# ketanfatania/QMRI-PnP-Recon-POC

Hardware: AMD Instinct MI355X
Metric: ADMM iters/sec (224x224x10 TSMI, spiral mask) (higher is better)
Workload: dtype f32; 1 GPU; cut3 224x224x10 single slice per GPU, spiral mask S=771 T=200, PnP-ADMM + 10-channel UNetRes (DRUNet) denoiser; solver=lsqr, admm_iters=20, dc_dtype=f64, parallelism=slice-parallel x1 (no collective)

## Files before the change

### qmri_pnp_recon_poc_amd/csrc/api_core.cpp

```cpp
#include "qmri_internal.h"
#include "fft_codelets.h"

#include <algorithm>
#include <atomic>
#include <cmath>
#include <cstdarg>
#include <cstdlib>
#include <cstring>
#include <mutex>

static thread_local std::string g_create_err;

namespace {
struct KnobDef { const char* name; int dflt; };
const KnobDef g_knob_defs[K_COUNT] = {
    {"conv_scheme", 2}, {"conv_f32", 0}, {"conv_wt", 1}, {"conv_xcd", 1}, {"conv_persist", 1}, {"conv_splitk", 1},
    {"conv_midcfg", 3}, {"conv_deepcfg", 3}, {"conv_deepks", 4},
    {"conv_resident", 1}, {"res_head", 1}, {"res_tail", 1}, {"res_down", 1}, {"res_delay", 24}, {"res_rearm", 64},
    {"res_stamps", 0}, {"conv_stamps", 0}, {"conv_stamp_launch", -1}, {"lsqr_stamps", 0},
    {"conv_mt2", 1024}, {"conv_occ", 2},
    {"fuse_ew", 1}, {"lsqr_persist", 1}, {"lsqr_fold", 1}, {"dictw_lsp", 2}, {"verbose", 0},
    {"pack_gpu", 1}, {"nufft_seg", NU_SEG},
};
std::atomic<int> g_knob_val[K_COUNT];
std::once_flag g_knob_once;

int knob_index(const char* name, size_t len) {
    for (int k = 0; k < K_COUNT; ++k)
        if (strlen(g_knob_defs[k].name) == len && strncmp(g_knob_defs[k].name, name, len) == 0) return k;
    return -1;
}
void knob_init() {
    for (int k = 0; k < K_COUNT; ++k) g_knob_val[k].store(g_knob_defs[k].dflt, std::memory_order_relaxed);
    const char* e = getenv("QMRI_DEBUG");
    while (e && *e) {
        const char* end = strchr(e, ',');
        const size_t len = end ? (size_t)(end - e) : strlen(e);
        const char* eq = (const char*)memchr(e, '=', len);
        const int k = eq ? knob_index(e, (size_t)(eq - e)) : -1;
        if (k >= 0) g_knob_val[k].store(atoi(eq + 1), std::memory_order_relaxed);
        else if (len) fprintf(stderr, "libqmri: QMRI_DEBUG: unknown or malformed entry '%.*s' ignored\n", (int)len, e);
// ... 829 lines not shown
```

### qmri_pnp_recon_poc_amd/csrc/api_net.cpp

```cpp
#include "qmri_internal.h"

#include <algorithm>
#include <cmath>
#include <cstdio>
#include <cstring>
#include <thread>
#include <chrono>
#include <cstdlib>

void qmri_free_operator(qmri_ctx* ctx);
int qmri_prepare_direct(qmri_ctx* ctx, double r);
int qmri_lsqr_run(qmri_ctx* ctx, int B, const double2* d_z, double r, double tol, int maxit, double2* d_x,
                  int32_t* iters_out, int32_t* flag_out, double* pdiag, LsqrState* hslot, bool* deferred, const LsqrFuse* fuse);

extern "C" size_t qmri_net_nparams(const qmri_net_desc* d) {
    if (!d) return 0;
    size_t n = 0;
    if (d->arch == QMRI_ARCH_UNETRES) {
        const int32_t* nc = d->nc;
        n += (size_t)nc[0] * d->in_nc * 9;
        for (int l = 0; l < 3; ++l) n += (size_t)2 * d->nb * nc[l] * nc[l] * 9 + (size_t)nc[l + 1] * nc[l] * 4;
        n += (size_t)2 * d->nb * nc[3] * nc[3] * 9;
        for (int l = 3; l > 0; --l) n += (size_t)nc[l] * nc[l - 1] * 4 + (size_t)2 * d->nb * nc[l - 1] * nc[l - 1] * 9;
        n += (size_t)d->out_nc * nc[0] * 9;
// ... 382 lines not shown
        for (int l = 0; l < 4; ++l) { p.x[l].blk = blk; p.a[l].blk = blk; p.t[l].blk = blk; }
    }
    const bool report = !ctx->net.force_f32;
    const bool timed = ctx->prof_level >= 2;
    if (timed) QMRI_HIP(ctx, hipEventRecord(ctx->ev[2], ctx->stream));
    if (report) QMRI_TRY(conv6_act_begin(ctx, (int)ctx->net.layers.size()));
    QMRI_TRY(net_forward_layers(ctx, B));
    if (report) QMRI_TRY(conv6_act_end(ctx));
    if (timed) QMRI_HIP(ctx, hipEventRecord(ctx->ev[3], ctx->stream));
    QMRI_TRY(qmri_prof_chain_finish(ctx));
    if (timed) {
        float ms = 0.f;
        QMRI_HIP(ctx, hipEventSynchronize(ctx->ev[3]));
        QMRI_HIP(ctx, hipEventElapsedTime(&ms, ctx->ev[2], ctx->ev[3]));
        ctx->prof.ms_net_forward += ms; ctx->prof.n_net_forward += 1;
    }
    return QMRI_OK;
}

static int net_forward_layers(qmri_ctx* ctx, int B) {
    NetPlan& p = ctx->net;
    const int nb = p.desc.nb;
    size_t li = 0;
    if (p.desc.arch == QMRI_ARCH_SEQ_CONV) {
        const size_t nl = p.layers.size();
        const PTensor* in = &p.in32;
        const PTensor* bufs[2] = { &p.a[0], &p.t[0] };
        for (size_t l = 0; l < nl; ++l) {
            const PTensor* out = (l == nl - 1) ? &p.out32 : bufs[l & 1];
            QMRI_TRY(run_conv(ctx, p.layers[l], B, *in, *out, nullptr, nullptr, l != nl - 1));
            in = out;
        }
        return QMRI_OK;
    }
    const bool res_head = qmri_knob(K_RES_HEAD) != 0, res_tail = qmri_knob(K_RES_TAIL) != 0, res_down = qmri_knob(K_RES_DOWN) != 0;
    bool head_done = false, down_done = false;
    if (res_head && p.d_res_xbuf && !p.force_f32 && p.layers.size() >= (size_t)(2 + 2 * nb)) {
        Conv6rRun r;
        r.head = &p.layers[0]; r.head_in = &p.in32; r.res = &p.layers[1]; r.nres = 2 * nb; r.src = &p.x[0]; r.cur = &p.a[0];
        if (res_down) {
            r.down = &p.layers[1 + 2 * nb]; r.down_out = &p.x[1];
            QMRI_TRY(conv6r_try(ctx, r, B, &down_done));
            if (down_done) { head_done = true; li = (size_t)(2 + 2 * nb); }
            r.down = nullptr; r.down_out = nullptr;
        }
        if (!down_done) {
            QMRI_TRY(conv6r_try(ctx, r, B, &head_done));
            if (head_done) li = (size_t)(1 + 2 * nb);
        }
    }
    if (!head_done) QMRI_TRY(run_conv(ctx, p.layers[li++], B, p.in32, p.x[0], nullptr, nullptr, 0));
    for (int l = 0; l < 3; ++l) {
        if (!(l == 0 && head_done)) QMRI_TRY(run_resblocks(ctx, li, nb, B, p.x[l], p.a[l], p.t[l], nullptr));
        if (!(l == 0 && down_done)) QMRI_TRY(run_conv(ctx, p.layers[li++], B, p.a[l], p.x[l + 1], nullptr, nullptr, 0));
    }
    QMRI_TRY(run_resblocks(ctx, li, nb, B, p.x[3], p.a[3], p.t[3], &p.x[3]));
    for (int l = 3; l > 0; --l) {
        QMRI_TRY(run_conv(ctx, p.layers[li++], B, p.a[l], p.a[l - 1], nullptr, nullptr, 0));
        if (l == 1 && res_tail && p.d_res_xbuf && !p.force_f32 && li + (size_t)(2 * nb) < p.layers.size()) {
            bool done = false;
            Conv6rRun r;
            r.res = &p.layers[li]; r.nres = 2 * nb; r.src = &p.a[0]; r.cur = &p.a[0]; r.skip = &p.x[0]; r.tail = &p.layers[li + 2 * nb]; r.tail_out = &p.out32;
            QMRI_TRY(conv6r_try(ctx, r, B, &done));
            if (done) { li += (size_t)(2 * nb + 1); return QMRI_OK; }
        }
        QMRI_TRY(run_resblocks(ctx, li, nb, B, p.a[l - 1], p.a[l - 1], p.t[l - 1], &p.x[l - 1]));
    }
    QMRI_TRY(run_conv(ctx, p.layers[li++], B, p.a[0], p.out32, nullptr, nullptr, 0));
    return QMRI_OK;
}

static int net_forward(qmri_ctx* ctx, int B) {
    NetPlan& p = ctx->net;
    const int st = net_forward_padded(ctx, B);
// ... 274 lines not shown
        QMRI_TRY(dc_launch_fwd(ctx, op, o.ls, DC_SPECTRUM, B, aty, o.d_tmp, o.d_chat, nullptr));
    } else if (prm->solver != QMRI_SOLVER_LSQR) {
        qmri_set_error(ctx, "unknown solver %d", prm->solver);
        return QMRI_ERR_INVALID_ARG;
    }
    if (prm->want_diag && diag_out) {
        if (o.d_diag) { (void)hipFree(o.d_diag); o.d_diag = nullptr; }
        QMRI_HIP(ctx, hipMalloc((void**)&o.d_diag, (size_t)B * std::max(prm->iters, 1) * 2 * sizeof(double)));
    }
    std::vector<int32_t> it_b(B);
    o.xhat_valid = false;
    const bool diag = prm->want_diag && diag_out;
    bool range_trip = false;
    std::vector<char> deferred_it((size_t)std::max(prm->iters, 1), 0);
    if (prm->solver == QMRI_SOLVER_LSQR && (size_t)prm->iters * B > o.h_ring_cap) {
        if (o.h_ring) { QMRI_HIP(ctx, hipStreamSynchronize(ctx->stream)); (void)hipHostFree(o.h_ring); o.h_ring = nullptr; o.h_ring_cap = 0; }
        const size_t cap = std::max<size_t>((size_t)prm->iters * B, 128);
        QMRI_HIP(ctx, hipHostMalloc((void**)&o.h_ring, cap * sizeof(LsqrState), hipHostMallocDefault));
        o.h_ring_cap = cap;
    }
    const bool fused = qmri_knob(K_FUSE_EW) != 0 && prm->solver == QMRI_SOLVER_LSQR;
    const int hb = dc_hpass_blocks(op);
    bool z_in_tmp = false;
    struct DeferGuard { NetPlan& n; ~DeferGuard() { n.act_defer = false; n.act_pending_valid = false; } } defer_guard{net};
    net.act_defer = fused;
    for (int it = 0; it < prm->iters; ++it) {
        tm.start();
        if (it == 0) QMRI_TRY(dc_launch_prepare_z(ctx, op, o.ls, B, o.d_vv, o.d_u, o.d_z));
        if (prm->solver == QMRI_SOLVER_LSQR) {
            bool deferred = false;
            LsqrFuse lf;
            if (fused) { lf.z_hpass_nblk = z_in_tmp ? hb : 0; lf.mm_u = o.d_u; lf.mm = o.d_mm; lf.mm_cpx = cpx; }
            QMRI_TRY(qmri_lsqr_run(ctx, B, o.d_z, prm->gamma, prm->cg_tol, prm->cg_maxit, o.d_x, it_b.data(), nullptr,
                                   diag ? o.d_pd : nullptr,
                                   o.h_ring + (size_t)it * B, &deferred, &lf));
            deferred_it[it] = deferred ? 1 : 0;
            if (!deferred && lsqr_iters_out) for (int b = 0; b < B; ++b) lsqr_iters_out[(size_t)b * prm->iters + it] = it_b[b];
            if (it > 0 && net.sp6 == 2 && host_range_tripped(net)) { range_trip = true; tm.stop(ctx->prof.ms_xupdate); break; }
        } else {
            QMRI_TRY(dc_launch_direct(ctx, op, B, o.d_z, o.d_chat, prm->gamma, o.d_tmp, o.d_x));
            if (lsqr_iters_out) for (int b = 0; b < B; ++b) lsqr_iters_out[(size_t)b * prm->iters + it] = 0;
        }
        tm.stop(ctx->prof.ms_xupdate);
        if (prm->want_diag && diag_out) {
            tm.start();
            if (prm->solver != QMRI_SOLVER_LSQR) QMRI_TRY(dc_launch_fwd(ctx, op, o.ls, DC_DIAG, B, o.d_x, o.d_tmp, nullptr, o.d_pd));
            QMRI_TRY(ew_launch_diag(ctx, op, o.ls, B, o.d_x, (const double2*)d_gt, o.d_pd, o.d_diag, prm->iters, it));
            tm.stop(ctx->prof.ms_diag);
        }
        tm.start();
        QMRI_TRY(ew_launch_minmax_normalise(ctx, B, n, (int)plane, o.N, o.s, multi, prm->noise_std, o.d_x, o.d_u, o.d_mm, o.d_norm,
                                            fused ? hb : o.ls.nblk_z, net.in32, fused , cpx));
        tm.stop(ctx->prof.ms_elementwise);
        tm.start();
        QMRI_TRY(net_forward(ctx, B));
        if (net.sp6 == 2 && (int)net.layers.size() + 1 > net.h_range_words)
            QMRI_HIP(ctx, hipMemcpyAsync(net.h_range_flag, net.d_range_flag, sizeof(unsigned), hipMemcpyDeviceToHost, ctx->stream));
        tm.stop(ctx->prof.ms_denoiser);
        tm.start();
        if (fused) {
            const DualArgs da = {net.out32.base1(), net.in32.base1(), net.out32.hp, (int)net.out32.plane(), net.out32.batch_stride(), net.in32.batch_stride(),
                                 net.desc.residual_noise, o.d_norm, o.d_x, o.d_u, o.ls.pz, cpx ? 1 : 0};
            ActCheckArgs ac{};
            if (net.act_pending_valid) { ac = net.act_pending; net.act_pending_valid = false; }
            QMRI_TRY(dc_launch_dual_fwd_h(ctx, op, B, da, ac, o.d_tmp));
            z_in_tmp = true;
        } else {
            QMRI_TRY(ew_launch_unnormalise_dual(ctx, B, n, (int)plane, o.N, net.out32, net.in32, net.desc.residual_noise, o.d_norm, o.d_x, o.d_u,
                                                nullptr , o.d_z, o.ls.pz, o.ls.nblk_z,
                                                o.s, cpx));
        }
        tm.stop(ctx->prof.ms_elementwise);
        ctx->prof.admm_iters += 1;
    }
    if (!range_trip) {
// ... 575 lines not shown
```

### qmri_pnp_recon_poc_amd/csrc/conv6r_kernels.hip

```cpp
#include "conv6_device.h"

namespace {

constexpr int R_MAXL = 10;
constexpr int R_RELU = 1;
constexpr int R_ADD = 2;
constexpr int R_SKIP = 4;
constexpr int R_STORE = 8;
constexpr int R_STORE_WT = 16;
constexpr int R_KEEP = 32;
constexpr int R_DOWN = 128;
constexpr unsigned R_DOWN_STEPB = 2 * 2 * 2 * 64 * 16;
constexpr int R_LOCAL = 256;
constexpr int R_TAIL = 64;
constexpr int R_IH = 18, R_IW = 18, R_IHP = 24;
constexpr int R_NPX = R_IHP * (R_IW - 1) + R_IH;
constexpr int R_CHUNK = 2 * 2 * R_NPX;
constexpr int R_AST = ast6(2);
constexpr int R_SPIN_MAX = 1 << 16;
constexpr int R_SEGT = 86, R_CORT = 6;
constexpr int R_NTRI = 4 * R_SEGT + 4 * R_CORT;
constexpr size_t conv6r_lds() { return (size_t)(NABUF * R_AST + 4 * R_CHUNK) * 16; }

struct Conv6rArgs {
    const float* src; const float* skip;
    const float* radd[R_MAXL]; float* sdst[R_MAXL];
    float* dn_out; int dn_hp, dn_plane;
    float* out; int out_hp, out_plane, out_c;
    int in_planar, in_plane;
    int nch[R_MAXL], kind[R_MAXL];
    unsigned char* xbuf; size_t xbuf_half;
    const uint4* wp[R_MAXL];
    float dh[R_MAXL], dl[R_MAXL];
    int am_layer[R_MAXL];
    int nlayers, hp, plane, tiles_h, tiles_w, xcd;
    int drop;
    int delay;
    unsigned epoch;
    unsigned* range_flag; float* am_slots; int* am_count;
    unsigned long long* stamps;
};

template <int N> __device__ __forceinline__ void gwait_a(u32x4 (&a)[3]) { asm volatile("s_waitcnt vmcnt(%3)" : "+v"(a[0]), "+v"(a[1]), "+v"(a[2]) : "n"(N) : "memory"); }
template <int IMM> __device__ __forceinline__ void gload4r_sc1(f32x4& dst, unsigned off, const void* base) { asm volatile("global_load_dwordx4 %0, %1, %2 offset:%3 sc1" : "=v"(dst) : "v"(off), "s"(base), "n"(IMM) : "memory"); }
template <int IMM> __device__ __forceinline__ void gstore4r(unsigned off, f32x4 x, void* base) { asm volatile("global_store_dwordx4 %0, %1, %2 offset:%3\n\ts_nop 1" ::"v"(off), "v"(x), "s"(base), "n"(IMM) : "memory"); }
template <int IMM> __device__ __forceinline__ void gstore4r_sc1(unsigned off, f32x4 x, void* base) { asm volatile("global_store_dwordx4 %0, %1, %2 offset:%3 sc1\n\ts_nop 1" ::"v"(off), "v"(x), "s"(base), "n"(IMM) : "memory"); }

__device__ __forceinline__ void r_tri_decode(int t, int& seg, int& j) {
    if (t < 4 * R_SEGT) { seg = t / R_SEGT; j = t - seg * R_SEGT; } else { seg = 4 + (t - 4 * R_SEGT) / R_CORT; j = (t - 4 * R_SEGT) - (seg - 4) * R_CORT; }
}
__device__ __forceinline__ int r_seg_base(int seg) { return seg < 4 ? seg * R_SEGT : 4 * R_SEGT + (seg - 4) * R_CORT; }
__device__ __forceinline__ unsigned r_ent_lds(int k, int dw, int dh) {
    const int cb = k >> 1, sp = k & 1;
    return (unsigned)(((cb >> 1) * R_CHUNK + sp * 2 * R_NPX + (cb & 1) * R_NPX + dw * R_IHP + dh) * 16);
}

#define R_STAMP(role, k)                                                                                         \
    do {                                                                                                         \
        if constexpr (STAMP) {                                                                                   \
            if (A.stamps && (threadIdx.x & 255) == 0 && blockIdx.x % 50 == 0 && blockIdx.x / 50 < 4)             \
                A.stamps[(((blockIdx.x / 50) * 2 + (role)) * R_MAXL + l) * 8 + (k)] = wall_clock64();            \
        }                                                                                                        \
    } while (0)
template <bool STAMP>
__global__ __launch_bounds__(NT6) void k_conv6r(const Conv6rArgs A) {
    constexpr int SP = 2, AST = R_AST, IHP = R_IHP, NPX = R_NPX, NAQ = 3;
    static_assert(AST == NAQ * NLD6, "one weight step = three 16-byte entries per loader thread");
    extern __shared__ __align__(16) unsigned char smem[];
    uint4* Abuf = (uint4*)smem;
// ... 39 lines not shown
                f32x4 v[NPRO];
                unsigned lo[NPRO];
#pragma unroll
                for (int k = 0; k < NPRO; ++k) {
                    const int idx = lt + NLD6 * k;
                    const bool valid = idx < NHALF;
                    const int idc = valid ? idx : 0, half = idc & 1, item = idc >> 1;
                    const int cb = item / (R_IH * R_IW), px = item - cb * (R_IH * R_IW), dw = px / R_IH, dh = px - dw * R_IH;
                    gload4r(v[k], (unsigned)cb * plane32 + (unsigned)((dw * A.hp + dh) * 32 + 16 * half) + tile0, A.src);
                    lo[k] = valid ? (unsigned)(((cb >> 1) * R_CHUNK + (cb & 1) * NPX + dw * IHP + dh) * 16 + 8 * half) : ~0u;
                }
                static_assert(NPRO == 21, "the wait below names 21 registers");
                asm volatile("s_waitcnt vmcnt(0)"
                             : "+v"(v[0]), "+v"(v[1]), "+v"(v[2]), "+v"(v[3]), "+v"(v[4]), "+v"(v[5]), "+v"(v[6]), "+v"(v[7]), "+v"(v[8]), "+v"(v[9]), "+v"(v[10]),
                               "+v"(v[11]), "+v"(v[12]), "+v"(v[13]), "+v"(v[14]), "+v"(v[15]), "+v"(v[16]), "+v"(v[17]), "+v"(v[18]), "+v"(v[19]), "+v"(v[20])::"memory");
#pragma unroll
                for (int k = 0; k < NPRO; ++k) {
                    uint2 s0, s1;
                    split_pair_h(v[k][0], v[k][1], s0.x, s1.x);
                    split_pair_h(v[k][2], v[k][3], s0.y, s1.y);
                    if (lo[k] != ~0u) {
                        *(uint2*)((unsigned char*)Bt + lo[k]) = s0;
                        *(uint2*)((unsigned char*)Bt + lo[k] + 2 * NPX * 16) = s1;
                    }
                }
            } else {
                constexpr int NIT = 2 * R_IH * R_IW, NQ = (NIT + NLD6 - 1) / NLD6;
                static_assert(NQ == 3, "the wait below names 24 registers");
                const int nin = A.nch[0];
                const unsigned pl4 = (unsigned)A.in_plane * 4u, t0 = (unsigned)((ow0 * A.hp + oh0) * 4);
#pragma unroll 1
                for (int ck = 0; ck < nin; ++ck) {
                    float v[NQ][8];
                    unsigned lo[NQ];
#pragma unroll
                    for (int k = 0; k < NQ; ++k) {
                        const int idx = lt + NLD6 * k;
                        const bool valid = idx < NIT;
                        const int idc = valid ? idx : 0, kh = idc / (R_IH * R_IW), px = idc - kh * (R_IH * R_IW), dw = px / R_IH, dh = px - dw * R_IH;
#pragma unroll
                        for (int j = 0; j < 8; ++j) gload1(v[k][j], (unsigned)(16 * ck + 8 * kh + j) * pl4 + (unsigned)((dw * A.hp + dh) * 4) + t0, A.src);
                        lo[k] = valid ? (unsigned)((ck * R_CHUNK + kh * NPX + dw * IHP + dh) * 16) : ~0u;
                    }
                    if (ck == 0) {
                        const uint4 z = make_uint4(0u, 0u, 0u, 0u);
                        for (int i = lt; i < (4 - nin) * R_CHUNK; i += NLD6) Bt[nin * R_CHUNK + i] = z;
// ... 401 lines not shown
}

}

int conv6r_try(qmri_ctx* ctx, const Conv6rRun& run, int B, bool* done) {
    *done = false;
    NetPlan& net = ctx->net;
    hipStreamCaptureStatus cap = hipStreamCaptureStatusNone;
    const bool capturing = hipStreamIsCapturing(ctx->stream, &cap) == hipSuccess && cap != hipStreamCaptureStatusNone;
    const int nres = run.nres, nl = nres + (run.head ? 1 : 0) + (run.tail ? 1 : 0) + (run.down ? 1 : 0);
    if (!qmri_knob(K_CONV_RESIDENT) || capturing || net.res_off || !net.d_res_xbuf || B != 1 || nres < 2 || nl > R_MAXL || (nres & 1) || net.d_stamps) return QMRI_OK;
    if (!run.res || !run.src || !run.cur || (run.head && (!run.head_in || run.skip)) || (run.tail && !run.tail_out) || (run.down && (!run.down_out || run.tail || run.skip))) return QMRI_OK;
    auto is3 = [](const ConvLayer& L) { return (L.kind == CONV_3X3 || L.kind == CONV_3X3N) && L.sp6 == 2 && L.wp6 && L.n_ct6 == 1; };
    for (int l = 0; l < nres; ++l) {
        const ConvLayer& L = run.res[l];
        if (!is3(L) || L.Cin != 64 || L.Cout != 64 || L.nchunk6 != 4) return QMRI_OK;
    }
    const PTensor &src = *run.src, &cur = *run.cur;
    const PTensor* ts[3] = {&src, &cur, run.skip};
    for (const PTensor* t : ts) {
        if (!t) continue;
        if (!t->p || !t->blk || t->Cal < 64 || t->H != src.H || t->W != src.W || t->hp != src.hp || t->h0 != src.h0) return QMRI_OK;
    }
    if (run.head) {
        const ConvLayer& L = *run.head;
        const PTensor& in = *run.head_in;
        if (!is3(L) || L.Cout != 64 || L.nchunk6 < 1 || L.nchunk6 > 2 || L.Cin > 16 * L.nchunk6 || !in.p || in.blk || in.Cal < 16 * L.nchunk6 || in.H != src.H || in.W != src.W || in.hp != src.hp ||
            in.h0 != src.h0 || src.p == cur.p) return QMRI_OK;
    }
    if (run.tail) {
        const ConvLayer& L = *run.tail;
        const PTensor& out = *run.tail_out;
        if (!is3(L) || L.Cin != 64 || L.nchunk6 != 4 || L.Cout > 32 || !out.p || out.blk || out.H != src.H || out.W != src.W ||
            (size_t)out.Cal * out.plane() * 4 >= ((size_t)1 << 31)) return QMRI_OK;
    }
    if (run.down) {
        const ConvLayer& L = *run.down;
        const PTensor& out = *run.down_out;
        if (L.kind != CONV_DOWN || L.sp6 != 2 || !L.wp6 || L.Cin != 64 || L.Cout != 128 || L.nchunk6 != 9 || L.n_ct6 != 2 || !out.p || !out.blk || out.Cal < 128 ||
            out.H * 2 != src.H || out.W * 2 != src.W || (size_t)out.Cal * out.plane() * 4 >= ((size_t)1 << 31)) return QMRI_OK;
    }
    if (src.H % 16 || src.W % 16) return QMRI_OK;
    if ((size_t)src.Cal * src.plane() * 4 >= ((size_t)1 << 31)) return QMRI_OK;
    if (!ctx->conv_ncu) {
        hipDeviceProp_t prop;
        QMRI_HIP(ctx, hipGetDeviceProperties(&prop, ctx->device));
        ctx->conv_ncu = prop.multiProcessorCount;
    }
    const int tiles_h = src.H / 16, tiles_w = src.W / 16, tiles = tiles_h * tiles_w;
    if (tiles > ctx->conv_ncu || tiles != net.res_tiles) return QMRI_OK;
    Conv6rArgs A{};
    A.src = run.head ? run.head_in->fbase() : src.fbase();
    A.in_planar = run.head ? 1 : 0; A.in_plane = run.head ? (int)run.head_in->plane() : 0;
    A.skip = run.skip ? run.skip->fbase() : nullptr;
    if (run.down) { A.dn_out = run.down_out->fbase(); A.dn_hp = run.down_out->hp; A.dn_plane = (int)run.down_out->plane(); }
    if (run.tail) { A.out = run.tail_out->fbase(); A.out_hp = run.tail_out->hp; A.out_plane = (int)run.tail_out->plane(); A.out_c = run.tail->Cout; }
    int l = 0;
    auto put = [&](const ConvLayer& L, int kind, const float* radd, float* sdst) {
        A.wp[l] = reinterpret_cast<const uint4*>(L.wp6);
        A.dh[l] = L.w6_descale; A.dl[l] = L.w6_descale * (1.f / LO_SCALE);
        A.am_layer[l] = conv6_act_slot(ctx, true, L).layer;
        A.nch[l] = L.nchunk6; A.kind[l] = kind; A.radd[l] = radd; A.sdst[l] = sdst;
        ++l;
    };
    if (run.head) put(*run.head, R_STORE | R_KEEP, nullptr, src.fbase());
    for (int r = 0; r < nres; ++r) {
        const bool last = r == nres - 1;
        if (!(r & 1)) put(run.res[r], R_RELU | R_KEEP, nullptr, nullptr);
        else if (!last) put(run.res[r], R_ADD | R_STORE | R_KEEP, (r == 1) ? src.fbase() : cur.fbase(), cur.fbase());
        else if (run.tail) put(run.res[r], R_ADD | (run.skip ? R_SKIP : 0) | R_KEEP, (r == 1) ? src.fbase() : cur.fbase(), nullptr);
        else if (run.down) put(run.res[r], R_ADD | R_KEEP | R_LOCAL, (r == 1) ? src.fbase() : cur.fbase(), nullptr);
        else put(run.res[r], R_ADD | (run.skip ? R_SKIP : 0) | R_STORE_WT, (r == 1) ? src.fbase() : cur.fbase(), cur.fbase());
    }
    if (run.tail) put(*run.tail, R_TAIL, nullptr, nullptr);
    if (run.down) { put(*run.down, R_DOWN, nullptr, nullptr); A.nch[l - 1] = 6; }
    for (int k = l; k < R_MAXL; ++k) { A.wp[k] = A.wp[l - 1]; A.nch[k] = A.nch[l - 1]; A.am_layer[k] = -1; }
    int pub[2] = {0, 0};
    for (int k = 0; k < l; ++k) if ((A.kind[k] & R_KEEP) && !(A.kind[k] & R_LOCAL)) pub[k & 1] += 1;
    if (!pub[0] || !pub[1]) return QMRI_OK;
    A.nlayers = nl; A.hp = src.hp; A.plane = (int)src.plane(); A.tiles_h = tiles_h; A.tiles_w = tiles_w;
    A.xbuf = net.d_res_xbuf; A.xbuf_half = (size_t)tiles * R_NTRI * 64;
    A.xcd = qmri_knob(K_CONV_XCD);
    const int delay = std::max(0, std::min(4096, qmri_knob(K_RES_DELAY)));
    A.epoch = net.res_epoch; A.drop = net.res_drop; A.delay = delay;
    A.range_flag = net.d_range_flag; A.am_slots = net.d_act_slots; A.am_count = net.d_act_count;
    if (!ctx->conv6r_attr) {
        QMRI_HIP(ctx, hipFuncSetAttribute((const void*)k_conv6r<false>, hipFuncAttributeMaxDynamicSharedMemorySize, (int)conv6r_lds()));
        QMRI_HIP(ctx, hipFuncSetAttribute((const void*)k_conv6r<true>, hipFuncAttributeMaxDynamicSharedMemorySize, (int)conv6r_lds()));
        ctx->conv6r_attr = true;
    }
    g_conv6_launch_counter.fetch_add(nl, std::memory_order_relaxed);
    const int stamp_which = qmri_knob(K_RES_STAMPS);
    A.stamps = (stamp_which == 2) == (run.head != nullptr) ? (unsigned long long*)net.d_res_stamps : nullptr;
    hipEvent_t e0 = nullptr, e1 = nullptr;
    double flop = 0.0;
    for (int r = 0; r < nres; ++r) flop += conv_layer_flop(run.res[r], 1, src.H, src.W);
    if (run.head) flop += conv_layer_flop(*run.head, 1, src.H, src.W);
    if (run.tail) flop += conv_layer_flop(*run.tail, 1, src.H, src.W);
    if (run.down) flop += conv_layer_flop(*run.down, 1, src.H, src.W);
    QMRI_TRY(qmri_prof_pair(ctx, &e0, &e1, PROF_CONV3, flop));
    if (A.stamps) k_conv6r<true><<<dim3(tiles), dim3(NT6), conv6r_lds(), ctx->stream>>>(A);
    else if (e0) hipExtLaunchKernelGGL((k_conv6r<false>), dim3(tiles), dim3(NT6), (std::uint32_t)conv6r_lds(), ctx->stream, e0, e1, 0, A);
    else k_conv6r<false><<<dim3(tiles), dim3(NT6), conv6r_lds(), ctx->stream>>>(A);
    QMRI_HIP(ctx, hipGetLastError());
    net.res_epoch += (unsigned)(nl - 1);
    *done = true;
    return QMRI_OK;
}

size_t conv6r_xbuf_bytes(int tiles) { return (size_t)2 * tiles * R_NTRI * 64; }
```

### qmri_pnp_recon_poc_amd/csrc/ew_kernels.hip

```cpp
#include "qmri_internal.h"

namespace {
__device__ __forceinline__ void st_wt(double2* p, double2 v) {
    typedef double d2v_ __attribute__((ext_vector_type(2)));
    const d2v_ t = {v.x, v.y};
    asm volatile("global_store_dwordx4 %0, %1, off sc1\n\ts_nop 1" ::"v"(p), "v"(t) : "memory");
}
}

namespace {

constexpr int NT = 256;

__device__ __forceinline__ double block_sum(double v, double* sh) {
#pragma unroll
    for (int off = 32; off > 0; off >>= 1) v += __shfl_down(v, off, 64);
    const int wid = threadIdx.x >> 6, lane = threadIdx.x & 63;
    __syncthreads();
    if (lane == 0) sh[wid] = v;
    __syncthreads();
    double r = 0.0;
#pragma unroll
    for (int i = 0; i < NT / 64; ++i) r += sh[i];
    return r;
// ... 204 lines not shown
    if (residual_noise) I = in32[(size_t)b * in_bs + pi] - I;
    out[(size_t)b * count + i] = (T)(I * scale);
}

__global__ __launch_bounds__(NT) void k_real_to_complex(size_t count, const double* __restrict__ in, double2* __restrict__ out) {
    const size_t i = (size_t)blockIdx.x * NT + threadIdx.x;
    if (i < count) out[i] = make_double2(in[i], 0.0);
}

}

int ew_launch_minmax_normalise(qmri_ctx* ctx, int B, size_t n, int plane, int H, int s, int multi_level, double noise_std,
                               const double2* x, const double2* u, double* mm, double* norm, int nblk, const PTensor& in32, bool mm_ready,
                               bool complex_tsmi) {
    auto go = [&](auto cpx) {
        constexpr bool CPX = decltype(cpx)::value;
        if (!mm_ready) k_minmax<CPX><<<dim3(nblk, B), dim3(NT), 0, ctx->stream>>>(n, x, u, mm);
        k_normalise<CPX><<<dim3(nblk, B), dim3(NT), 0, ctx->stream>>>(n, plane, H, s, multi_level, noise_std, x, u, mm, nblk, norm, in32.base1(),
                                                                      in32.hp, (int)in32.plane(), in32.batch_stride());
    };
    if (complex_tsmi) go(std::true_type{});
    else go(std::false_type{});
    QMRI_HIP(ctx, hipGetLastError());
    return QMRI_OK;
}

int ew_launch_unnormalise_dual(qmri_ctx* ctx, int B, size_t n, int plane, int H, const PTensor& out32, const PTensor& in32,
                               int residual_noise, const double* norm, const double2* x, double2* u, double2* v, double2* z,
                               double* pz, int nblk_z, int s, bool complex_tsmi) {
    auto go = [&](auto cpx) {
        k_unnormalise_dual<decltype(cpx)::value><<<dim3(nblk_z, B), dim3(NT), 0, ctx->stream>>>(
            n, plane, H, s, out32.hp, (int)out32.plane(), out32.batch_stride(), in32.batch_stride(), out32.base1(), in32.base1(), residual_noise,
            norm, x, u, v, z, pz);
    };
    if (complex_tsmi) go(std::true_type{});
    else go(std::false_type{});
    QMRI_HIP(ctx, hipGetLastError());
    return QMRI_OK;
}

int ew_launch_diag(qmri_ctx* ctx, const OpDev& op, const LsqrDev& ls, int B, const double2* x, const double2* gt,
                   double* pd, double* diag_slot, int iters_total, int it) {
    const size_t n = (size_t)op.s * op.N * op.M;
    double* pg = pd + (size_t)B * op.N;
    if (gt) k_diffnorm<<<dim3(ls.nblk_z, B), dim3(NT), 0, ctx->stream>>>(n, gt, x, pg);
    k_diag_final<<<dim3(B), dim3(NT), 0, ctx->stream>>>(ls.st, pd, op.N, pg, ls.nblk_z, gt ? 1 : 0, diag_slot, iters_total, it);
    QMRI_HIP(ctx, hipGetLastError());
// ... 80 lines not shown
```

### qmri_pnp_recon_poc_amd/csrc/qmri_internal.h

```cpp
#pragma once

#include <hip/hip_runtime.h>
#include <cstdint>
#include <cstdio>
#include <string>
#include <vector>

#include "../../include/qmri.h"

struct qmri_ctx;
void qmri_set_error(qmri_ctx* ctx, const char* fmt, ...);

#define QMRI_HIP(ctx, expr)                                                                       \
    do {                                                                                          \
        hipError_t _e = (expr);                                                                   \
        if (_e != hipSuccess) {                                                                   \
            qmri_set_error((ctx), "%s failed: %s (%s:%d)", #expr, hipGetErrorString(_e), __FILE__, __LINE__); \
            return QMRI_ERR_HIP;                                                                  \
        }                                                                                         \
    } while (0)

#define QMRI_CHECK_ARG(ctx, cond, msg)                                                            \
    do {                                                                                          \
        if (!(cond)) {                                                                            \
            qmri_set_error((ctx), "invalid argument: %s", (msg));                                 \
            return QMRI_ERR_INVALID_ARG;                                                          \
        }                                                                                         \
    } while (0)

#define QMRI_TRY(expr)                                                                            \
    do {                                                                                          \
        int _s = (expr);                                                                          \
        if (_s != QMRI_OK) return _s;                                                             \
    } while (0)

enum QmriKnob {
    K_CONV_SCHEME,
    K_CONV_F32,
    K_CONV_WT,
    K_CONV_XCD,
    K_CONV_PERSIST,
    K_CONV_SPLITK,
    K_CONV_MIDCFG, K_CONV_DEEPCFG, K_CONV_DEEPKS,
    K_CONV_RESIDENT,
    K_RES_HEAD, K_RES_TAIL, K_RES_DOWN,
    K_RES_DELAY,
    K_RES_REARM,
    K_RES_STAMPS, K_CONV_STAMPS, K_CONV_STAMP_LAUNCH, K_LSQR_STAMPS,
    K_CONV_MT2, K_CONV_OCC,
    K_FUSE_EW,
    K_LSQR_PERSIST,
    K_LSQR_FOLD,
    K_DICTW_LSP,
    K_VERBOSE,
    K_PACK_GPU,
    K_NUFFT_SEG,
    K_COUNT
};
int qmri_knob(QmriKnob k);

struct KEntry {
    uint16_t kw;
    uint16_t t;
};


struct OpDev {
    int N, M, s, T, m;
// ... 76 lines not shown
    int tab_B, tab_MT;
    void* wp6 = nullptr;
    int sp6 = 2;
    float w6_descale = 1.f;
    int nchunk6 = 0, n_ct6 = 0;
    int nsteps6s = 0;
    int index = -1;
    size_t w_off = 0;
};

struct PTensor {
    float* p = nullptr;
    int C = 0, Cal = 0, H = 0, W = 0;
    int hp = 0, h0 = 1;
    bool blk = false;
    float* base1() const { return p + (h0 - 1); }
    float* fbase() const { return p + (size_t)(h0 - 1) * (blk ? 8 : 1); }
    size_t plane() const { return (size_t)hp * (W + 2); }
    size_t batch_stride() const { return (size_t)Cal * plane(); }
};

struct ActCheckArgs { const float* slots; int* count; float* ref; int record; unsigned* range_flag; unsigned* host_words; int nlayers; };

struct NetPlan {
    qmri_net_desc desc{};
    int H = 0, W = 0, maxB = 0;
    std::vector<ConvLayer> layers;
    PTensor x[4], a[4], t[4];
    PTensor in32;
    PTensor out32;
    std::vector<float*> allocs;
    unsigned* d_counter = nullptr;
    unsigned counter_base = 0;
    bool counter_by_memset = false;
    bool force_f32 = false;
    unsigned* d_range_flag = nullptr;
    unsigned* h_range_flag = nullptr;
    int h_range_words = 0;
    int fallbacks = 0;
    float* d_act_slots = nullptr;
    int* d_act_count = nullptr;
    float* d_act_ref = nullptr;
    int act_cap = 0;
    bool act_on = false, act_record = false;
    bool act_defer = false, act_pending_valid = false;
    ActCheckArgs act_pending{};
    int sp6 = 2;
    bool blk_ok = false;
    int interior_fmt = -1;
    std::vector<float> w_host;
    float* d_wflat = nullptr;
    const float* w_begin = nullptr;
    std::vector<float> w_max;
    float* d_c6part = nullptr;
    size_t c6part_floats = 0;
    void* d_stamps = nullptr;
    unsigned char* d_res_xbuf = nullptr;
    int res_tiles = 0;
    unsigned res_epoch = 0;
    bool res_off = false;
    bool res_forced_off = false;
    double setup_ms[3] = {0, 0, 0};
    int res_timeouts = 0;
    int res_clean = 0;
    int res_drop = 0;
    double* d_io = nullptr; size_t io_cap = 0;
    void* d_res_stamps = nullptr;
    bool ready = false;
};
// ... 166 lines not shown
struct DualArgs {
    const float* out32; const float* in32; int php, pplane; size_t out_bs, in_bs; int residual_noise;
    const double* norm; const double2* x; double2* u; double* pz;
    int complex_tsmi;
};
int dc_hpass_blocks(const OpDev& op);
struct LsqrFuse { int z_hpass_nblk = 0; const double2* mm_u = nullptr; double* mm = nullptr; bool mm_cpx = false; };
int dc_launch_dual_fwd_h(qmri_ctx* ctx, const OpDev& op, int B, const DualArgs& d, const ActCheckArgs& ac, double2* tmp);
int ks_launch_init(qmri_ctx* ctx, const OpDev& op, const KsDev& ks, int B, const double2* hpass_tmp = nullptr, bool first_step = true);
int ks_launch_iter(qmri_ctx* ctx, const OpDev& op, const KsDev& ks, int B);
int ks_launch_final(qmri_ctx* ctx, const OpDev& op, const KsDev& ks, int B, double2* tmp);
int ks_persist_plan(qmri_ctx* ctx, const OpDev& op, const KsDev& ks, int B, int* per_launch);
int ks_launch_persist(qmri_ctx* ctx, const OpDev& op, const KsDev& ks, int B, void* gran, unsigned tag0, bool init_here, bool* ran);
size_t ks_gran_bytes(int G, int B);
int ks_lds_fits(qmri_ctx* ctx, int N, int s, int M, int vcap, int caps, bool* ok);
int dc_launch_direct(qmri_ctx* ctx, const OpDev& op, int B, const double2* z, const double2* chat, double r,
                     double2* tmp, double2* x_out);
int dc_launch_sort_y(qmri_ctx* ctx, const OpDev& op, const LsqrDev& ls, int B, const double2* y);
int dc_launch_prepare_z(qmri_ctx* ctx, const OpDev& op, const LsqrDev& ls, int B, const double2* v, const double2* u,
                        double2* z);
int ew_launch_minmax_normalise(qmri_ctx* ctx, int B, size_t n, int plane, int H, int s, int multi_level, double noise_std,
                               const double2* x, const double2* u, double* mm, double* norm, int nblk, const PTensor& in32, bool mm_ready = false,
                               bool complex_tsmi = false);
int ew_launch_unnormalise_dual(qmri_ctx* ctx, int B, size_t n, int plane, int H, const PTensor& out32, const PTensor& in32,
                               int residual_noise, const double* norm, const double2* x, double2* u, double2* v, double2* z,
                               double* pz, int nblk_z, int s = 0, bool complex_tsmi = false);
int ew_launch_diag(qmri_ctx* ctx, const OpDev& op, const LsqrDev& ls, int B, const double2* x, const double2* gt,
                   double* pd, double* diag_slot, int iters_total, int it);
int ew_launch_pack(qmri_ctx* ctx, int B, int C, int H, int W, const void* src, int src_is_double, const PTensor& dst, float scale = 1.f);
int ew_launch_absmax(qmri_ctx* ctx, const float* x, const float* y, size_t n, unsigned* d_out);
int ew_launch_unpack(qmri_ctx* ctx, int B, int C, int H, int W, const PTensor& out32, const PTensor& in32, int residual_noise,
                     void* dst, int dst_is_double, float scale = 1.f);
int ew_launch_real_to_complex(qmri_ctx* ctx, size_t count, const double* in, double2* out);
int ew_launch_coil_mul(qmri_ctx* ctx, size_t n, size_t plane, int cnt, const double2* x, const double2* maps, double2* out);
int ew_launch_coil_sum(qmri_ctx* ctx, size_t n, size_t plane, int cnt, const double2* xj, const double2* maps, double2* x, int accumulate);

int conv_launch(qmri_ctx* ctx, ConvLayer& L, int B, const PTensor& in, const PTensor& out, const PTensor* add1,
                const PTensor* add2, int relu_out);
int conv_cin_pad(ConvKind kind, int Cin);
enum { PROF_CONV3 = 0, PROF_CONV2 = 1, PROF_LSQR = 2, PROF_TV = 3 };
int qmri_prof_pair(qmri_ctx* ctx, hipEvent_t* start, hipEvent_t* stop, int kind = PROF_CONV3, double flop = 0.0);
int qmri_prof_chain_finish(qmri_ctx* ctx, long count = -1);
bool conv6_enabled();
int conv6_act_begin(qmri_ctx* ctx, int nlayers);
int conv6_act_end(qmri_ctx* ctx);
int conv6_default_sp();
bool conv6_weights_fit_f16(const float* w, size_t n);
void conv6_plan_pack(ConvLayer& L, const float* w, std::vector<uint16_t>& packed);
int conv6_pack_dev(qmri_ctx* ctx, ConvLayer& L, const float* d_w, float wmax);
int conv6s_pack_dev(qmri_ctx* ctx, ConvLayer& L, const float* d_w, float wmax);
int conv_pack_weights_dev(qmri_ctx* ctx, ConvLayer& L, const float* d_w);
int conv6_launch(qmri_ctx* ctx, const ConvLayer& L, int B, const PTensor& in, const PTensor& out, const PTensor* add1,
                 const PTensor* add2, int relu_out);
struct Conv6rRun {
    const ConvLayer* head = nullptr; const PTensor* head_in = nullptr;
    const ConvLayer* res = nullptr; int nres = 0;
    const PTensor* src = nullptr; const PTensor* cur = nullptr; const PTensor* skip = nullptr;
    const ConvLayer* tail = nullptr; const PTensor* tail_out = nullptr;
    const ConvLayer* down = nullptr; const PTensor* down_out = nullptr;
};
int conv6r_try(qmri_ctx* ctx, const Conv6rRun& run, int B, bool* done);
size_t conv6r_xbuf_bytes(int tiles);
void conv6s_plan_pack(ConvLayer& L, const float* w, std::vector<uint16_t>& packed);
bool conv6s_usable(const ConvLayer& L, const PTensor& in, const PTensor& out);
int conv6s_launch(qmri_ctx* ctx, const ConvLayer& L, int B, const PTensor& in, const PTensor& out);
size_t conv_pack_weights(const ConvLayer& L, const float* w_src, std::vector<float>& packed);
void conv_plan_layer(ConvLayer& L, ConvKind kind, int Cin, int Cout);

int dict_launch(qmri_ctx* ctx, const double2* d_X, int Npix, float* d_qmap, float* d_pd, float* d_mt, int32_t* d_dm, float2* d_xfit);
int dict_scratch(qmri_ctx* ctx, void** buf, size_t* cap, size_t need_bytes);
int dict_launch_merge(qmri_ctx* ctx, const float4* part, int P, int Npix, float* d_qmap, float* d_pd, float* d_mt, int32_t* d_dm, float4* win);
int dictw_pack_dictionary(qmri_ctx* ctx, const float* D_host, int K, int s);
int dictw_launch(qmri_ctx* ctx, const double2* d_X, int Npix, float* d_qmap, float* d_pd, float* d_mt, int32_t* d_dm, float4* win);
```

Before: 818.0 ADMM iters/s.

## Fold min-max normalisation into resident head conv kernel input staging

Instead of launching a separate min-max normalise kernel that writes the f32 network input, the per-iteration normalise parameters are deferred and consumed by the resident conv6r head kernel, which reduces the block min/max partials, reads x+u in f64 directly, normalises and packs into its LDS tile. This removes one kernel launch and one round trip of the normalised input through global memory per ADMM iteration. Every block redundantly reduces the min/max partials, and there is a fallback path that launches the normalise alone when the fold is not possible.

```diff
diff --git a/qmri_pnp_recon_poc_amd/csrc/api_core.cpp b/qmri_pnp_recon_poc_amd/csrc/api_core.cpp
--- a/qmri_pnp_recon_poc_amd/csrc/api_core.cpp
+++ b/qmri_pnp_recon_poc_amd/csrc/api_core.cpp
@@ -16,7 +16,7 @@
 const KnobDef g_knob_defs[K_COUNT] = {
     {"conv_scheme", 2}, {"conv_f32", 0}, {"conv_wt", 1}, {"conv_xcd", 1}, {"conv_persist", 1}, {"conv_splitk", 1},
     {"conv_midcfg", 3}, {"conv_deepcfg", 3}, {"conv_deepks", 4},
-    {"conv_resident", 1}, {"res_head", 1}, {"res_tail", 1}, {"res_down", 1}, {"res_delay", 24}, {"res_rearm", 64},
+    {"conv_resident", 1}, {"res_head", 1}, {"res_tail", 1}, {"res_down", 1}, {"res_norm", 1}, {"res_delay", 24}, {"res_rearm", 64},
     {"res_stamps", 0}, {"conv_stamps", 0}, {"conv_stamp_launch", -1}, {"lsqr_stamps", 0},
     {"conv_mt2", 1024}, {"conv_occ", 2},
     {"fuse_ew", 1}, {"lsqr_persist", 1}, {"lsqr_fold", 1}, {"dictw_lsp", 2}, {"verbose", 0},
diff --git a/qmri_pnp_recon_poc_amd/csrc/api_net.cpp b/qmri_pnp_recon_poc_amd/csrc/api_net.cpp
--- a/qmri_pnp_recon_poc_amd/csrc/api_net.cpp
+++ b/qmri_pnp_recon_poc_amd/csrc/api_net.cpp
@@ -428,7 +428,11 @@
     NetPlan& p = ctx->net;
     const int nb = p.desc.nb;
     size_t li = 0;
+    const bool norm_waits = p.norm_pending_valid;
+    p.norm_pending_valid = false;
+    auto normalise_alone = [&]() -> int { return norm_waits ? ew_launch_normalise(ctx, B, p.norm_pending, p.in32) : QMRI_OK; };
     if (p.desc.arch == QMRI_ARCH_SEQ_CONV) {
+        QMRI_TRY(normalise_alone());
         const size_t nl = p.layers.size();
         const PTensor* in = &p.in32;
         const PTensor* bufs[2] = { &p.a[0], &p.t[0] };
@@ -444,6 +448,7 @@
     if (res_head && p.d_res_xbuf && !p.force_f32 && p.layers.size() >= (size_t)(2 + 2 * nb)) {
         Conv6rRun r;
         r.head = &p.layers[0]; r.head_in = &p.in32; r.res = &p.layers[1]; r.nres = 2 * nb; r.src = &p.x[0]; r.cur = &p.a[0];
+        r.norm = norm_waits ? &p.norm_pending : nullptr;
         if (res_down) {
             r.down = &p.layers[1 + 2 * nb]; r.down_out = &p.x[1];
             QMRI_TRY(conv6r_try(ctx, r, B, &down_done));
@@ -455,7 +460,10 @@
             if (head_done) li = (size_t)(1 + 2 * nb);
         }
     }
-    if (!head_done) QMRI_TRY(run_conv(ctx, p.layers[li++], B, p.in32, p.x[0], nullptr, nullptr, 0));
+    if (!head_done) {
+        QMRI_TRY(normalise_alone());
+        QMRI_TRY(run_conv(ctx, p.layers[li++], B, p.in32, p.x[0], nullptr, nullptr, 0));
+    }
     for (int l = 0; l < 3; ++l) {
         if (!(l == 0 && head_done)) QMRI_TRY(run_resblocks(ctx, li, nb, B, p.x[l], p.a[l], p.t[l], nullptr));
         if (!(l == 0 && down_done)) QMRI_TRY(run_conv(ctx, p.layers[li++], B, p.a[l], p.x[l + 1], nullptr, nullptr, 0));
@@ -776,8 +784,10 @@
     const bool fused = qmri_knob(K_FUSE_EW) != 0 && prm->solver == QMRI_SOLVER_LSQR;
     const int hb = dc_hpass_blocks(op);
     bool z_in_tmp = false;
-    struct DeferGuard { NetPlan& n; ~DeferGuard() { n.act_defer = false; n.act_pending_valid = false; } } defer_guard{net};
+    struct DeferGuard { NetPlan& n; ~DeferGuard() { n.act_defer = false; n.act_pending_valid = false; n.norm_pending_valid = false; } } defer_guard{net};
     net.act_defer = fused;
+    const bool norm_fold = fused && B == 1 && qmri_knob(K_RES_NORM) != 0 && qmri_knob(K_RES_HEAD) != 0 && !net.desc.residual_noise && ctx->prof_level < 2 &&
+                           net.desc.in_nc == (cpx ? 2 * o.s : o.s) + multi;
     for (int it = 0; it < prm->iters; ++it) {
         tm.start();
         if (it == 0) QMRI_TRY(dc_launch_prepare_z(ctx, op, o.ls, B, o.d_vv, o.d_u, o.d_z));
@@ -803,8 +813,13 @@
             tm.stop(ctx->prof.ms_diag);
         }
         tm.start();
-        QMRI_TRY(ew_launch_minmax_normalise(ctx, B, n, (int)plane, o.N, o.s, multi, prm->noise_std, o.d_x, o.d_u, o.d_mm, o.d_norm,
-                                            fused ? hb : o.ls.nblk_z, net.in32, fused , cpx));
+        if (norm_fold) {
+            net.norm_pending = NormArgs{n, (int)plane, o.N, o.s, multi, hb, prm->noise_std, o.d_x, o.d_u, o.d_mm, o.d_norm, cpx};
+            net.norm_pending_valid = true;
+        } else {
+            QMRI_TRY(ew_launch_minmax_normalise(ctx, B, n, (int)plane, o.N, o.s, multi, prm->noise_std, o.d_x, o.d_u, o.d_mm, o.d_norm,
+                                                fused ? hb : o.ls.nblk_z, net.in32, fused , cpx));
+        }
         tm.stop(ctx->prof.ms_elementwise);
         tm.start();
         QMRI_TRY(net_forward(ctx, B));
diff --git a/qmri_pnp_recon_poc_amd/csrc/conv6r_kernels.hip b/qmri_pnp_recon_poc_amd/csrc/conv6r_kernels.hip
--- a/qmri_pnp_recon_poc_amd/csrc/conv6r_kernels.hip
+++ b/qmri_pnp_recon_poc_amd/csrc/conv6r_kernels.hip
@@ -28,6 +28,8 @@
     float* dn_out; int dn_hp, dn_plane;
     float* out; int out_hp, out_plane, out_c;
     int in_planar, in_plane;
+    const double2* nx; const double2* nu; const double* nmm; double* nnorm; double n_noise;
+    int n_nblk, n_s, n_multi, n_cpx, n_h, n_plane;
     int nch[R_MAXL], kind[R_MAXL];
     unsigned char* xbuf; size_t xbuf_half;
     const uint4* wp[R_MAXL];
@@ -45,6 +47,12 @@
 template <int IMM> __device__ __forceinline__ void gload4r_sc1(f32x4& dst, unsigned off, const void* base) { asm volatile("global_load_dwordx4 %0, %1, %2 offset:%3 sc1" : "=v"(dst) : "v"(off), "s"(base), "n"(IMM) : "memory"); }
 template <int IMM> __device__ __forceinline__ void gstore4r(unsigned off, f32x4 x, void* base) { asm volatile("global_store_dwordx4 %0, %1, %2 offset:%3\n\ts_nop 1" ::"v"(off), "v"(x), "s"(base), "n"(IMM) : "memory"); }
 template <int IMM> __device__ __forceinline__ void gstore4r_sc1(unsigned off, f32x4 x, void* base) { asm volatile("global_store_dwordx4 %0, %1, %2 offset:%3 sc1\n\ts_nop 1" ::"v"(off), "v"(x), "s"(base), "n"(IMM) : "memory"); }
+
+__device__ __forceinline__ double r_first(double v) {
+    const unsigned long long b = __builtin_bit_cast(unsigned long long, v);
+    const unsigned lo = __builtin_amdgcn_readfirstlane((unsigned)b), hi = __builtin_amdgcn_readfirstlane((unsigned)(b >> 32));
+    return __builtin_bit_cast(double, ((unsigned long long)hi << 32) | lo);
+}
 
 __device__ __forceinline__ void r_tri_decode(int t, int& seg, int& j) {
     if (t < 4 * R_SEGT) { seg = t / R_SEGT; j = t - seg * R_SEGT; } else { seg = 4 + (t - 4 * R_SEGT) / R_CORT; j = (t - 4 * R_SEGT) - (seg - 4) * R_CORT; }
@@ -130,6 +138,103 @@
                     if (lo[k] != ~0u) {
                         *(uint2*)((unsigned char*)Bt + lo[k]) = s0;
                         *(uint2*)((unsigned char*)Bt + lo[k] + 2 * NPX * 16) = s1;
+                    }
+                }
+            } else if (A.nx) {
+                constexpr int NIT = 2 * R_IH * R_IW, NQ = (NIT + NLD6 - 1) / NLD6;
+                static_assert(NQ == 3, "the waits below name 2 x 24 registers");
+                const int nin = A.nch[0], ns = A.n_s, nreal = A.n_cpx ? 2 * ns : ns;
+                const int img_w = A.tiles_w * 16, img_h = A.tiles_h * 16;
+                const float noise = (float)A.n_noise;
+#pragma unroll 1
+                for (int ck = 0; ck < nin; ++ck) {
+                    double xv[NQ][8], uv[NQ][8];
+                    unsigned lo[NQ], live[NQ];
+#pragma unroll
+                    for (int k = 0; k < NQ; ++k) {
+                        const int idx = lt + NLD6 * k;
+                        const bool valid = idx < NIT;
+                        const int idc = valid ? idx : 0, kh = idc / (R_IH * R_IW), px = idc - kh * (R_IH * R_IW), dw = px / R_IH, dh = px - dw * R_IH;
+                        const int gw = ow0 + dw - 1, gh = oh0 + dh - 1;
+                        const bool inside = valid && gw >= 0 && gw < img_w && gh >= 0 && gh < img_h;
+                        const unsigned pix = inside ? (unsigned)((gw * A.n_h + gh) * 16) : 0u;
+                        live[k] = 0u;
+#pragma unroll
+                        for (int j = 0; j < 8; ++j) {
+                            const int ch = 16 * ck + 8 * kh + j;
+                            const bool data = inside && ch < nreal;
+                            const int sc = data ? (ch < ns ? ch : ch - ns) : 0;
+                            const unsigned off = (unsigned)sc * ((unsigned)A.n_plane * 16u) + pix + ((data && ch >= ns) ? 8u : 0u);
+                            asm volatile("global_load_dwordx2 %0, %1, %2" : "=v"(xv[k][j]) : "v"(off), "s"(A.nx) : "memory");
+                            asm volatile("global_load_dwordx2 %0, %1, %2" : "=v"(uv[k][j]) : "v"(off), "s"(A.nu) : "memory");
+                            live[k] |= data ? (1u << j) : 0u;
+                            if (inside && ch == nreal && A.n_multi) live[k] |= 1u << (8 + j);
+                        }
+                        lo[k] = valid ? (unsigned)((ck * R_CHUNK + kh * NPX + dw * IHP + dh) * 16) : ~0u;
+                    }
+                    if (ck == 0) {
+                        const uint4 z = make_uint4(0u, 0u, 0u, 0u);
+                        for (int i = lt; i < (4 - nin) * R_CHUNK; i += NLD6) Bt[nin * R_CHUNK + i] = z;
+                    }
+                    double mn, range;
+                    {
+                        const int ln = lt & 63;
+                        double wl[4], wh[4];
+#pragma unroll
+                        for (int v = 0; v < 4; ++v) { wl[v] = INFINITY; wh[v] = -INFINITY; }
+                        for (int i0 = ln; i0 < A.n_nblk; i0 += 256) {
+                            double pl[4], ph[4];
+#pragma unroll
+                            for (int v = 0; v < 4; ++v) {
+                                const int i = i0 + 64 * v, ic = (i < A.n_nblk) ? i : i0;
+                                pl[v] = A.nmm[2 * ic]; ph[v] = A.nmm[2 * ic + 1];
+                                if (i >= A.n_nblk) { pl[v] = INFINITY; ph[v] = -INFINITY; }
+                            }
+#pragma unroll
+                            for (int v = 0; v < 4; ++v) { wl[v] = fmin(wl[v], pl[v]); wh[v] = fmax(wh[v], ph[v]); }
+                        }
+#pragma unroll
+                        for (int off = 32; off > 0; off >>= 1) {
+                            double sl[4], sh[4];
+#pragma unroll
+                            for (int v = 0; v < 4; ++v) { sl[v] = __shfl_down(wl[v], off, 64); sh[v] = __shfl_down(wh[v], off, 64); }
+#pragma unroll
+                            for (int v = 0; v < 4; ++v) { wl[v] = fmin(wl[v], sl[v]); wh[v] = fmax(wh[v], sh[v]); }
+                        }
+#pragma unroll
+                        for (int v = 0; v < 4; ++v) { wl[v] = r_first(wl[v]); wh[v] = r_first(wh[v]); }
+                        double hi = wh[0];
+                        mn = wl[0];
+#pragma unroll
+                        for (int v = 1; v < 4; ++v) { mn = fmin(mn, wl[v]); hi = fmax(hi, wh[v]); }
+                        range = hi - mn;
+                        if (ck == 0 && bid == 0 && lt == 0) { A.nnorm[0] = mn; A.nnorm[1] = range; }
+                    }
+                    asm volatile("s_waitcnt vmcnt(0)"
+                                 : "+v"(xv[0][0]), "+v"(xv[0][1]), "+v"(xv[0][2]), "+v"(xv[0][3]), "+v"(xv[0][4]), "+v"(xv[0][5]), "+v"(xv[0][6]), "+v"(xv[0][7]), "+v"(xv[1][0]),
+                                   "+v"(xv[1][1]), "+v"(xv[1][2]), "+v"(xv[1][3]), "+v"(xv[1][4]), "+v"(xv[1][5]), "+v"(xv[1][6]), "+v"(xv[1][7]), "+v"(xv[2][0]), "+v"(xv[2][1]),
+                                   "+v"(xv[2][2]), "+v"(xv[2][3]), "+v"(xv[2][4]), "+v"(xv[2][5]), "+v"(xv[2][6]), "+v"(xv[2][7])::"memory");
+                    asm volatile("s_waitcnt vmcnt(0)"
+                                 : "+v"(uv[0][0]), "+v"(uv[0][1]), "+v"(uv[0][2]), "+v"(uv[0][3]), "+v"(uv[0][4]), "+v"(uv[0][5]), "+v"(uv[0][6]), "+v"(uv[0][7]), "+v"(uv[1][0]),
+                                   "+v"(uv[1][1]), "+v"(uv[1][2]), "+v"(uv[1][3]), "+v"(uv[1][4]), "+v"(uv[1][5]), "+v"(uv[1][6]), "+v"(uv[1][7]), "+v"(uv[2][0]), "+v"(uv[2][1]),
+                                   "+v"(uv[2][2]), "+v"(uv[2][3]), "+v"(uv[2][4]), "+v"(uv[2][5]), "+v"(uv[2][6]), "+v"(uv[2][7])::"memory");
+#pragma unroll
+                    for (int k = 0; k < NQ; ++k) {
+                        float f[8];
+#pragma unroll
+                        for (int j = 0; j < 8; ++j) {
+                            const float d = (float)(((xv[k][j] + uv[k][j]) - mn) / range);
+                            f[j] = (live[k] >> j & 1u) ? d : ((live[k] >> (8 + j) & 1u) ? noise : 0.f);
+                        }
+                        uint4 s0, s1;
+                        split_pair_h(f[0], f[1], s0.x, s1.x);
+                        split_pair_h(f[2], f[3], s0.y, s1.y);
+                        split_pair_h(f[4], f[5], s0.z, s1.z);
+                        split_pair_h(f[6], f[7], s0.w, s1.w);
+                        if (lo[k] != ~0u) {
+                            *(uint4*)((unsigned char*)Bt + lo[k]) = s0;
+                            *(uint4*)((unsigned char*)Bt + lo[k] + 2 * NPX * 16) = s1;
+                        }
                     }
                 }
             } else {
@@ -577,9 +682,12 @@
         if (!t) continue;
         if (!t->p || !t->blk || t->Cal < 64 || t->H != src.H || t->W != src.W || t->hp != src.hp || t->h0 != src.h0) return QMRI_OK;
     }
+    if (run.norm && (!run.head || run.norm->H != src.H || (size_t)run.norm->plane != (size_t)src.H * src.W || run.norm->n != (size_t)run.norm->plane * run.norm->s ||
+                     run.norm->n * sizeof(double2) >= ((size_t)1 << 31) || run.norm->nblk < 1)) return QMRI_OK;
     if (run.head) {
         const ConvLayer& L = *run.head;
         const PTensor& in = *run.head_in;
+        if (run.norm && L.Cin != (run.norm->cpx ? 2 : 1) * run.norm->s + (run.norm->multi_level ? 1 : 0)) return QMRI_OK;
         if (!is3(L) || L.Cout != 64 || L.nchunk6 < 1 || L.nchunk6 > 2 || L.Cin > 16 * L.nchunk6 || !in.p || in.blk || in.Cal < 16 * L.nchunk6 || in.H != src.H || in.W != src.W || in.hp != src.hp ||
             in.h0 != src.h0 || src.p == cur.p) return QMRI_OK;
     }
@@ -608,6 +716,11 @@
     A.src = run.head ? run.head_in->fbase() : src.fbase();
     A.in_planar = run.head ? 1 : 0; A.in_plane = run.head ? (int)run.head_in->plane() : 0;
     A.skip = run.skip ? run.skip->fbase() : nullptr;
+    if (run.norm) {
+        const NormArgs& N = *run.norm;
+        A.nx = N.x; A.nu = N.u; A.nmm = N.mm; A.nnorm = N.norm; A.n_noise = N.noise_std;
+        A.n_nblk = N.nblk; A.n_s = N.s; A.n_multi = N.multi_level ? 1 : 0; A.n_cpx = N.cpx ? 1 : 0; A.n_h = N.H; A.n_plane = N.plane;
+    }
     if (run.down) { A.dn_out = run.down_out->fbase(); A.dn_hp = run.down_out->hp; A.dn_plane = (int)run.down_out->plane(); }
     if (run.tail) { A.out = run.tail_out->fbase(); A.out_hp = run.tail_out->hp; A.out_plane = (int)run.tail_out->plane(); A.out_c = run.tail->Cout; }
     int l = 0;
@@ -645,6 +758,7 @@
         ctx->conv6r_attr = true;
     }
     g_conv6_launch_counter.fetch_add(nl, std::memory_order_relaxed);
+    if (run.norm) g_normalise_folded.fetch_add(1, std::memory_order_relaxed);
     const int stamp_which = qmri_knob(K_RES_STAMPS);
     A.stamps = (stamp_which == 2) == (run.head != nullptr) ? (unsigned long long*)net.d_res_stamps : nullptr;
     hipEvent_t e0 = nullptr, e1 = nullptr;
diff --git a/qmri_pnp_recon_poc_amd/csrc/ew_kernels.hip b/qmri_pnp_recon_poc_amd/csrc/ew_kernels.hip
--- a/qmri_pnp_recon_poc_amd/csrc/ew_kernels.hip
+++ b/qmri_pnp_recon_poc_amd/csrc/ew_kernels.hip
@@ -250,7 +250,19 @@
     if (complex_tsmi) go(std::true_type{});
     else go(std::false_type{});
     QMRI_HIP(ctx, hipGetLastError());
-    return QMRI_OK;
+    g_normalise_launched.fetch_add(1, std::memory_order_relaxed);
+    return QMRI_OK;
+}
+
+std::atomic<long long> g_normalise_launched{0}, g_normalise_folded{0};
+extern "C" int qmri_test_normalise_counts(long long* launched_out, long long* folded_out) {
+    if (launched_out) *launched_out = g_normalise_launched.load(std::memory_order_relaxed);
+    if (folded_out) *folded_out = g_normalise_folded.load(std::memory_order_relaxed);
+    return QMRI_OK;
+}
+
+int ew_launch_normalise(qmri_ctx* ctx, int B, const NormArgs& a, const PTensor& in32) {
+    return ew_launch_minmax_normalise(ctx, B, a.n, a.plane, a.H, a.s, a.multi_level, a.noise_std, a.x, a.u, a.mm, a.norm, a.nblk, in32, true, a.cpx);
 }
 
 int ew_launch_unnormalise_dual(qmri_ctx* ctx, int B, size_t n, int plane, int H, const PTensor& out32, const PTensor& in32,
diff --git a/qmri_pnp_recon_poc_amd/csrc/qmri_internal.h b/qmri_pnp_recon_poc_amd/csrc/qmri_internal.h
--- a/qmri_pnp_recon_poc_amd/csrc/qmri_internal.h
+++ b/qmri_pnp_recon_poc_amd/csrc/qmri_internal.h
@@ -1,6 +1,7 @@
 #pragma once
 
 #include <hip/hip_runtime.h>
+#include <atomic>
 #include <cstdint>
 #include <cstdio>
 #include <string>
@@ -44,6 +45,7 @@
     K_CONV_MIDCFG, K_CONV_DEEPCFG, K_CONV_DEEPKS,
     K_CONV_RESIDENT,
     K_RES_HEAD, K_RES_TAIL, K_RES_DOWN,
+    K_RES_NORM,
     K_RES_DELAY,
     K_RES_REARM,
     K_RES_STAMPS, K_CONV_STAMPS, K_CONV_STAMP_LAUNCH, K_LSQR_STAMPS,
@@ -166,6 +168,11 @@
 
 struct ActCheckArgs { const float* slots; int* count; float* ref; int record; unsigned* range_flag; unsigned* host_words; int nlayers; };
 
+struct NormArgs {
+    size_t n = 0; int plane = 0, H = 0, s = 0, multi_level = 0, nblk = 0; double noise_std = 0.0;
+    const double2* x = nullptr; const double2* u = nullptr; double* mm = nullptr; double* norm = nullptr; bool cpx = false;
+};
+
 struct NetPlan {
     qmri_net_desc desc{};
     int H = 0, W = 0, maxB = 0;
@@ -189,6 +196,8 @@
     bool act_on = false, act_record = false;
     bool act_defer = false, act_pending_valid = false;
     ActCheckArgs act_pending{};
+    bool norm_pending_valid = false;
+    NormArgs norm_pending{};
     int sp6 = 2;
     bool blk_ok = false;
     int interior_fmt = -1;
@@ -401,6 +410,9 @@
 int ew_launch_minmax_normalise(qmri_ctx* ctx, int B, size_t n, int plane, int H, int s, int multi_level, double noise_std,
                                const double2* x, const double2* u, double* mm, double* norm, int nblk, const PTensor& in32, bool mm_ready = false,
                                bool complex_tsmi = false);
+int ew_launch_normalise(qmri_ctx* ctx, int B, const NormArgs& a, const PTensor& in32);
+extern "C" int qmri_test_normalise_counts(long long* launched_out, long long* folded_out);
+extern std::atomic<long long> g_normalise_launched, g_normalise_folded;
 int ew_launch_unnormalise_dual(qmri_ctx* ctx, int B, size_t n, int plane, int H, const PTensor& out32, const PTensor& in32,
                                int residual_noise, const double* norm, const double2* x, double2* u, double2* v, double2* z,
                                double* pz, int nblk_z, int s = 0, bool complex_tsmi = false);
@@ -433,6 +445,7 @@
                  const PTensor* add2, int relu_out);
 struct Conv6rRun {
     const ConvLayer* head = nullptr; const PTensor* head_in = nullptr;
+    const NormArgs* norm = nullptr;
     const ConvLayer* res = nullptr; int nres = 0;
     const PTensor* src = nullptr; const PTensor* cur = nullptr; const PTensor* skip = nullptr;
     const ConvLayer* tail = nullptr; const PTensor* tail_out = nullptr;
```

Measured after the change: 823.1 ADMM iters/s (median of 3 runs). About the same (+0.6%).
